# JamesYang007/adelie

Hardware: AMD Instinct MI355X
Metric: lambda-paths/sec (100-lambda grpnet); HBM GB/s vs peak (higher is better)
Workload: dtype f64

## Files before the change

adelie_amd/csrc/kernels.hpp:

```cpp
#pragma once
#include <hip/hip_runtime.h>
#include <cstdint>

namespace ahip {

template <class T>
struct DenseView {
    const T* X;
    int64_t n, p, ld;
};
struct SnpView {
    const uint8_t* bits;
    int64_t n, p, ldb;
};

template <class T>
struct CscView {
    const int64_t* cptr;
    const int32_t* cidx;
    const T* cval;
    const int64_t* rptr;
    const int32_t* rcol;
    const T* rval;
    int64_t n, p, nnz;
// ... 102 lines not shown
    int32_t moff[MAX], m[MAX], noff[MAX], nn[MAX];
    int64_t dst[MAX];
    int32_t count;
};
int64_t gram_batch_work_elems(int64_t n, int count);
template <class T>
void launch_gram_batch(const DenseView<T>& X, const T* w, const int32_t* cols_base, const GramBatch& b, const T* xm_by_col,
                       bool center, T* C_base, int64_t ldc, T* work, hipStream_t s);
template <class T>
void launch_gram_batch_snp(const SnpView& X, const T* impute, const T* w, const int32_t* cols_base, const GramBatch& b,
                           const T* xm_by_col, bool center, T* C_base, int64_t ldc, T* work, hipStream_t s);
struct StripBatch {
    static constexpr int MAX = 8;
    int32_t voff[MAX], m[MAX], c0off[MAX], c0n[MAX], c1off[MAX], c1n[MAX], row0[MAX];
    int64_t dstX[MAX], dstD[MAX];
    int32_t count;
};
int strip_row_tiles(int m);
int64_t strip_work_elems(int64_t n, int count, int m_max);
void set_strip_workgroups(int wgs);
void set_strip_lds(bool on);
template <class T>
void launch_strip_batch(const DenseView<T>& X, const T* w, const int32_t* cols_base, const StripBatch& b, const T* xm_by_col,
                        bool center, T* D_base, T* X_base, int64_t ldc, T* work, hipStream_t s);
void set_small_gram_workgroups(int wgs);
template <class T>
void launch_syrk_batch(const DenseView<T>& X, const T* w, const int32_t* cols_base, const SyrkBatch& b, const T* xm_by_col,
                       bool center, T* C_base, int64_t ldc, T* work, hipStream_t s);
template <class T>
void launch_syrk_batch_snp(const SnpView& X, const T* impute, const T* w, const int32_t* cols_base, const SyrkBatch& b,
                           const T* xm_by_col, bool center, T* C_base, int64_t ldc, T* work, hipStream_t s);
template <class T>
void launch_syrk(const DenseView<T>& X, const T* w, const int32_t* cols, int32_t M, const T* xm_by_col, bool center, T* C,
                   int64_t ldc, T* work, hipStream_t s);
template <class T>
void launch_syrk_snp(const SnpView& X, const T* impute, const T* w, const int32_t* cols, int32_t M, const T* xm_by_col,
                       bool center, T* C, int64_t ldc, T* work, hipStream_t s);
int64_t syrk_work_elems(int64_t n, int64_t M);

template <class T>
void launch_abs_grad(const T* grad, const int64_t* groups, const int64_t* group_sizes, int64_t G, const int32_t* slot,
                     const T* screen_beta, const T* penalty, T one_minus_alpha_lmda, T* abs_grad, hipStream_t s);
template <class T>
void launch_abs_grad_cons(const T* grad, const int64_t* groups, const int64_t* group_sizes, int64_t G, const int32_t* slot, const T* screen_beta,
                          const T* penalty, T one_minus_alpha_lmda, const T* clo, const T* chi, const T* cmu, T* abs_grad,
                          T* mu_out, hipStream_t s);

// ... 212 lines not shown
int launch_panel_step(const DenseView<T>& X, const T* w, T* r, const int32_t* dcol, const T* dlt, const int32_t* nz_dev,
                      const int32_t* cols, int nb, T* part, hipStream_t s);
template <class T>
struct StepTail {
    int32_t* counter;
    int32_t base;
    T* g;
    const T* rsum;
    const T* xm;
};
template <class T>
int launch_panel_step_snp(const SnpView& X, const T* impute, const T* w, T* r, const int32_t* dcol, const T* dlt,
                          const int32_t* nz_dev, const int32_t* cols, int nb, T* part, hipStream_t s,
                          const StepTail<T>* tail = nullptr, bool* tailed = nullptr);
int64_t panel_part_elems(int64_t n);
template <class T>
void launch_la_open_from_grad(const T* grad, const int32_t* cols, int nb, T* g, const T* rsum_src, T* rsum_out, hipStream_t s);
template <class T>
void launch_panel_reduce(const T* part, int nslices, int nb, const int32_t* cols, const T* rsum_dev, const T* xm_by_col,
                         T* gblk, hipStream_t s);
template <class T>
void launch_panel_reduce_ld(const T* part, int64_t part_ld, int nslices, int nb, const int32_t* cols, const T* rsum_dev,
                            const T* xm_by_col, T* gblk, hipStream_t s);
template <class T>
int launch_panel_fused(const CdBlkParams<T>& sp, int j, const DenseView<T>& X, const T* w, T* r, const int32_t* dcol,
                       const T* dlt, const int32_t* nz_dev, const int32_t* cols, int nb, T* part, bool tr, hipStream_t s);
template <class T>
int launch_panel_fused_snp(const CdBlkParams<T>& sp, int j, const SnpView& X, const T* impute, const T* w, T* r,
                           const int32_t* dcol, const T* dlt, const int32_t* nz_dev, const int32_t* cols, int nb, T* part,
                           bool tr, hipStream_t s);
template <class T>
int launch_panel_fused_grp(const CdGrpBlkParams<T>& sp, int j, const DenseView<T>& X, const T* w, T* r, const int32_t* dcol,
                           const T* dlt, const int32_t* nz_dev, const int32_t* cols, int nb, T* part, bool tr, hipStream_t s);
template <class T>
int launch_panel_fused_grp_snp(const CdGrpBlkParams<T>& sp, int j, const SnpView& X, const T* impute, const T* w, T* r,
                               const int32_t* dcol, const T* dlt, const int32_t* nz_dev, const int32_t* cols, int nb,
                               T* part, bool tr, hipStream_t s);
template <class T> void launch_cd_panel_solve(const CdBlkParams<T>& p, int j, hipStream_t s);
template <class T> void launch_center_vars(T* vars, const T* xm, int cnt, bool center, hipStream_t s);
void launch_gather_i32(const int32_t* src, const int32_t* idx, int cnt, int32_t* out, hipStream_t s);
template <class T>
void launch_cd_compact(const T* beta, const T* beta0, const int32_t* vcol, int nv, int32_t* dcols, T* dvals,
                       int32_t* n_delta, hipStream_t s);

template <class T>
struct MultiView {
// ... 138 lines not shown
```

adelie_amd/csrc/kernels_cd_panel.hip:

```cpp
#include "kernels.hpp"
#include "accessors.hpp"
#include "wavered.hpp"
#include "blk_solve_body.hpp"
#include "grp_solve_body.hpp"

namespace ahip {

namespace {

constexpr int PB = 128;
constexpr int PT = 256;

template <class T, int VEC>
struct RawDense { Pack<T, VEC> v; };
struct RawSnp { unsigned byte; };

template <class T, int VEC>
__device__ __forceinline__ RawDense<T, VEC> praw(const DenseAcc<T>& X, int64_t j, int64_t i, int64_t n, bool full) {
    RawDense<T, VEC> r;
    const T* col = X.colptr(j);
    if constexpr (VEC == 1) {
        const T x = col[(full || i < n) ? i : 0];
        r.v.v[0] = (full || i < n) ? x : T(0);
    } else {
// ... 420 lines not shown
            const T* b0 = reinterpret_cast<const T*>(smem_raw);
            const int c = threadIdx.x;
            const T tot = (b0[c] + b0[size_t(5) * RS + c]) + (b0[size_t(10) * RS + c] + b0[size_t(15) * RS + c]);
            T* dst = part + (part_ld > 0 ? int64_t(c) * part_ld + grp : grp * PB + c);
            if (coh) __hip_atomic_store(dst, tot, __ATOMIC_RELAXED, __HIP_MEMORY_SCOPE_AGENT);
            else *dst = tot;
        }
    } else {
        const int64_t slice4 = grp * FS + sub;
        if ((grp + 1) * FS * RS <= n)
            panel_step_body<T, Acc, VEC, true>(X, n, w, r, dcol, dlt, nz, cols, nb, part, part_ld, red, wrs, tid, slice4);
        else
            panel_step_body<T, Acc, VEC, false>(X, n, w, r, dcol, dlt, nz, cols, nb, part, part_ld, red, wrs, tid, slice4);
    }
}

inline int fused_fsa(int64_t ns) {
    if ((ns + 3) / 4 > 250) return 4;
    if (ns <= 250) return 1;
    if ((ns + 1) / 2 <= 250) return 2;
    return 4;
}

template <class T, class Acc, int VEC>
__global__ __launch_bounds__(256 * FS) void panel_fused_kernel(CdBlkParams<T> sp, int j, Acc X, int64_t n,
                                                              const T* __restrict__ w, T* __restrict__ r,
                                                              const int32_t* __restrict__ dcol, const T* __restrict__ dlt,
                                                              const int32_t* __restrict__ nz_dev,
                                                              const int32_t* __restrict__ cols, int nb,
                                                              T* __restrict__ part, int64_t part_ld, int fsa) {
    extern __shared__ __attribute__((aligned(16))) char smem_raw[];
    constexpr int RS = 64 * VEC;
    if (blockIdx.x == 0) {
        if (j < 0) {
            if (threadIdx.x == 0 && sp.part_rsum) {
                const T v = sp.part_rsum[0];
                sp.rsum_out[0] = v;
                sp.rsum_out[1] = v;
            }
            return;
        }
        blk_solve_la_body<T>(sp, j, smem_raw, threadIdx.x);
        return;
    }
    fused_step_part<T, Acc, VEC>(smem_raw, X, n, w, r, dcol, dlt, nz_dev, cols, nb, part, part_ld, fsa);
}
// ... 100 lines not shown
            }
            red[q * PB + c] = sacc;
        }
        __syncthreads();
        if (int(threadIdx.x) < cpw && c < nb) {
            T g = ((red[c] + red[PB + c]) + (red[2 * PB + c] + red[3 * PB + c])) +
                  ((red[4 * PB + c] + red[5 * PB + c]) + (red[6 * PB + c] + red[7 * PB + c]));
            if (sp.tail_xm) g -= sp.tail_rsum[0] * sp.tail_xm[cols[c]];
            sp.tail_g[c] = g;
        }
        if (threadIdx.x == 0) {
            const int d = __hip_atomic_fetch_add(sp.tail_counter + 1, 1, __ATOMIC_RELAXED, __HIP_MEMORY_SCOPE_AGENT);
            if (d == NT - 1) {
                __hip_atomic_store(sp.tail_counter + 1, 0, __ATOMIC_RELAXED, __HIP_MEMORY_SCOPE_AGENT);
                __hip_atomic_store(sp.tail_counter, 0, __ATOMIC_RELAXED, __HIP_MEMORY_SCOPE_AGENT);
            }
        }
    }
}

template <class T, class Acc, int VEC>
int fused_grp_launch(const CdGrpBlkParams<T>& sp, int j, const Acc& acc, int64_t n, const T* w, T* r, const int32_t* dcol,
                     const T* dlt, const int32_t* nz_dev, const int32_t* cols, int nb, T* part, bool tr, hipStream_t s) {
    constexpr int RS = 64 * VEC;
    const int64_t ns = (n + RS - 1) / RS;
    const int fsa = (64 * VEC >= PB) ? fused_fsa(ns) : FS;
    const int64_t nwg = (ns + fsa - 1) / fsa;
    const int64_t part_ld = (64 * VEC >= PB) ? nwg : nwg * FS;
    static bool attr_done = false;
    if (!attr_done) {
        (void)hipFuncSetAttribute(reinterpret_cast<const void*>(panel_fused_grp_kernel<T, Acc, VEC>),
                                  hipFuncAttributeMaxDynamicSharedMemorySize, int(grp_solve_lds_total<T>()));
        attr_done = true;
    }
    hipLaunchKernelGGL((panel_fused_grp_kernel<T, Acc, VEC>), dim3((unsigned)(nwg + 1)), dim3(256 * FS),
                       grp_solve_lds_total<T>(), s, sp, j, acc, n, w, r, dcol, dlt, nz_dev, cols, nb, part,
                       tr ? int64_t(0) : part_ld, fsa);
    return int(part_ld);
}

template <class T, class Acc, int VEC>
int fused_launch(const CdBlkParams<T>& sp, int j, const Acc& acc, int64_t n, const T* w, T* r, const int32_t* dcol,
                 const T* dlt, const int32_t* nz_dev, const int32_t* cols, int nb, T* part, bool tr, hipStream_t s) {
    constexpr int RS = 64 * VEC;
    const int64_t ns = (n + RS - 1) / RS;
    const int fsa = (64 * VEC >= PB) ? fused_fsa(ns) : FS;
    const int64_t nwg = (ns + fsa - 1) / fsa;
    const int64_t part_ld = (64 * VEC >= PB) ? nwg : nwg * FS;
    static bool attr_done = false;
    if (!attr_done) {
        (void)hipFuncSetAttribute(reinterpret_cast<const void*>(panel_fused_kernel<T, Acc, VEC>),
                                  hipFuncAttributeMaxDynamicSharedMemorySize, int(fused_lds<T>()));
        attr_done = true;
    }
    hipLaunchKernelGGL((panel_fused_kernel<T, Acc, VEC>), dim3((unsigned)(nwg + 1)), dim3(256 * FS),
                       fused_lds<T>(), s, sp, j, acc, n, w, r, dcol, dlt, nz_dev, cols, nb, part,
                       tr ? int64_t(0) : part_ld, fsa);
    return int(part_ld);
}

}

template <class T>
int launch_panel_fused(const CdBlkParams<T>& sp, int j, const DenseView<T>& X, const T* w, T* r, const int32_t* dcol,
                       const T* dlt, const int32_t* nz_dev, const int32_t* cols, int nb, T* part, bool tr, hipStream_t s) {
    DenseAcc<T> acc{X.X, X.ld};
    constexpr int V = VecOf<T>::N;
    const bool vecok = (X.ld % V == 0) && ((reinterpret_cast<uintptr_t>(X.X) % 16) == 0);
    if (vecok) return fused_launch<T, DenseAcc<T>, V>(sp, j, acc, X.n, w, r, dcol, dlt, nz_dev, cols, nb, part, tr, s);
    return fused_launch<T, DenseAcc<T>, 1>(sp, j, acc, X.n, w, r, dcol, dlt, nz_dev, cols, nb, part, tr, s);
}
template <class T>
int launch_panel_fused_snp(const CdBlkParams<T>& sp, int j, const SnpView& X, const T* impute, const T* w, T* r,
                           const int32_t* dcol, const T* dlt, const int32_t* nz_dev, const int32_t* cols, int nb, T* part,
                           bool tr, hipStream_t s) {
    SnpAcc<T> acc{X.bits, X.ldb, impute};
    return fused_launch<T, SnpAcc<T>, 4>(sp, j, acc, X.n, w, r, dcol, dlt, nz_dev, cols, nb, part, tr, s);
}

template <class T>
int launch_panel_fused_grp(const CdGrpBlkParams<T>& sp, int j, const DenseView<T>& X, const T* w, T* r, const int32_t* dcol,
                           const T* dlt, const int32_t* nz_dev, const int32_t* cols, int nb, T* part, bool tr, hipStream_t s) {
    DenseAcc<T> acc{X.X, X.ld};
// ... 118 lines not shown
```

adelie_amd/csrc/kernels_strip.hip:

```cpp
#include "gram_common.hpp"
#include "common.hpp"
#include <type_traits>

namespace ahip {

namespace {

constexpr int SGT = 256;
constexpr int SKC = 4;
constexpr int SCH = 4 * SKC;
constexpr int STG = 4;
constexpr int SW = 256;

template <class T, class Acc, bool VECOK, int MT, int TGL>
__device__ __forceinline__ void strip_wave(const Acc& X, const T* __restrict__ w, const int32_t* __restrict__ cols_base,
                                           const StripBatch& b, int y, int wv, int lane, int64_t k0, int64_t k1,
                                           T* __restrict__ P) {
    const int fr = lane & 15, fq = lane >> 4;
    const int m = b.m[y], c0n = b.c0n[y], ncol = c0n + b.c1n[y];
    const T* pa[MT];
    const T* pb[TGL];
    int64_t ja[MT], jb[TGL];
#pragma unroll
    for (int i = 0; i < MT; ++i) {
// ... 98 lines not shown
}

template <class T, class Acc, bool VECOK, int MT>
__global__ __launch_bounds__(SGT, (MT <= 2 ? 2 : 1)) void strip_kernel(Acc X, const T* __restrict__ w,
                                                                      const int32_t* __restrict__ cols_base, StripBatch b,
                                                                      int64_t n, int64_t kchunk, int nsplit,
                                                                      T* __restrict__ part) {
    const int y = blockIdx.y, sp = blockIdx.x;
    const int lane = threadIdx.x & 63;
    const int wv = __builtin_amdgcn_readfirstlane(int(threadIdx.x >> 6));
    const int ncol = b.c0n[y] + b.c1n[y];
    const int tg_live = min(STG, (ncol - wv * 64 + 15) >> 4);
    if (tg_live <= 0 || b.m[y] <= 0) return;
    const int64_t k0 = int64_t(sp) * kchunk, k1 = min(n, k0 + kchunk);
    if (k0 >= k1) return;
    T* P = part + (int64_t(y) * nsplit + sp) * (16 * MT) * SW;
    if (tg_live == 4) strip_wave<T, Acc, VECOK, MT, 4>(X, w, cols_base, b, y, wv, lane, k0, k1, P);
    else if (tg_live == 3) strip_wave<T, Acc, VECOK, MT, 3>(X, w, cols_base, b, y, wv, lane, k0, k1, P);
    else if (tg_live == 2) strip_wave<T, Acc, VECOK, MT, 2>(X, w, cols_base, b, y, wv, lane, k0, k1, P);
    else strip_wave<T, Acc, VECOK, MT, 1>(X, w, cols_base, b, y, wv, lane, k0, k1, P);
}

constexpr int SLP = 18;

template <class Acc, int MT, int TGL>
__device__ __forceinline__ void strip_wave_lt(const Acc& X, const double* __restrict__ w, const int32_t* __restrict__ cols_base,
                                              const StripBatch& b, int y, int wv, int lane, int64_t k0, int64_t k1,
                                              double* __restrict__ P, double* __restrict__ L) {
    using T = double;
    constexpr int NF = MT + TGL;
    const int fr = lane & 15, fq = lane >> 4;
    const int lc = lane >> 3, lp = lane & 7;
    const int m = b.m[y], c0n = b.c0n[y], ncol = c0n + b.c1n[y];
    const T* pg[NF][2];
    int64_t jg[NF][2];
#pragma unroll
    for (int f = 0; f < NF; ++f)
#pragma unroll
        for (int h = 0; h < 2; ++h) {
            const int c16 = h * 8 + lc;
            int64_t j;
            if (f < MT) {
                j = int64_t(cols_base[b.voff[y] + min(f * 16 + c16, m - 1)]);
            } else {
                const int c = min(wv * 64 + (f - MT) * 16 + c16, ncol - 1);
                j = int64_t(c < c0n ? cols_base[b.c0off[y] + c] : cols_base[b.c1off[y] + c - c0n]);
            }
            jg[f][h] = j;
            pg[f][h] = X.colptr(j) + lp * 2;
        }
    typename Mfma<T>::acc_t acc[MT][TGL];
#pragma unroll
    for (int i = 0; i < MT; ++i)
#pragma unroll
        for (int t = 0; t < TGL; ++t)
#pragma unroll
            for (int e = 0; e < 4; ++e) acc[i][t][e] = T(0);

    T g[NF][2][2], fv[NF][SKC], rw[SKC], rwn[SKC];
    auto fetch = [&](int64_t k) {
#pragma unroll
        for (int f = 0; f < NF; ++f)
#pragma unroll
            for (int h = 0; h < 2; ++h) {
                const Pack<T, 2> x = X.template load<2>(pg[f][h], k, jg[f][h]);
                g[f][h][0] = x.v[0];
                g[f][h][1] = x.v[1];
            }
#pragma unroll
        for (int u = 0; u < 2; ++u)
#pragma unroll
            for (int e = 0; e < 2; ++e) rwn[u * 2 + e] = w[k + u * 8 + fq * 2 + e];
    };
    typedef double d2_t __attribute__((ext_vector_type(2)));
    auto park = [&]() {
#pragma unroll
        for (int f = 0; f < NF; ++f)
#pragma unroll
            for (int h = 0; h < 2; ++h) {
                d2_t v = {g[f][h][0], g[f][h][1]};
                *reinterpret_cast<d2_t*>(L + (f * 16 + h * 8 + lc) * SLP + lp * 2) = v;
            }
#pragma unroll
        for (int e = 0; e < SKC; ++e) rw[e] = rwn[e];
    };
    auto frags = [&]() {
#pragma unroll
        for (int f = 0; f < NF; ++f)
#pragma unroll
            for (int u = 0; u < 2; ++u) {
                const d2_t v = *reinterpret_cast<const d2_t*>(L + (f * 16 + fr) * SLP + u * 8 + fq * 2);
                fv[f][u * 2] = v[0];
                fv[f][u * 2 + 1] = v[1];
            }
    };
    auto run = [&]() {
#pragma unroll
        for (int e = 0; e < SKC; ++e) {
            T a[MT];
#pragma unroll
            for (int i = 0; i < MT; ++i) a[i] = fv[i][e] * rw[e];
#pragma unroll
            for (int i = 0; i < MT; ++i)
#pragma unroll
                for (int t = 0; t < TGL; ++t) acc[i][t] = Mfma<T>::run(a[i], fv[MT + t][e], acc[i][t]);
        }
    };
    const int64_t kfull = k0 + ((k1 - k0) / SCH) * SCH;
    int64_t k = k0;
    if (k < kfull) {
        fetch(k);
        while (k < kfull) {
            park();
            fetch((k + 2 * SCH <= kfull) ? k + SCH : k);
            __builtin_amdgcn_fence(__ATOMIC_RELEASE, "wavefront");
            __builtin_amdgcn_wave_barrier();
            __builtin_amdgcn_fence(__ATOMIC_ACQUIRE, "wavefront");
            frags();
            __builtin_amdgcn_fence(__ATOMIC_RELEASE, "wavefront");
            __builtin_amdgcn_wave_barrier();
            run();
            k += SCH;
        }
    }
    if (k < k1) {
#pragma unroll
        for (int u = 0; u < 2; ++u)
#pragma unroll
            for (int e = 0; e < 2; ++e) {
                const int64_t kk = k + u * 8 + fq * 2 + e;
                const bool in = kk < k1;
#pragma unroll
                for (int f = 0; f < NF; ++f) {
                    int64_t j;
                    if (f < MT) {
                        j = int64_t(cols_base[b.voff[y] + min(f * 16 + fr, m - 1)]);
                    } else {
                        const int c = min(wv * 64 + (f - MT) * 16 + fr, ncol - 1);
                        j = int64_t(c < c0n ? cols_base[b.c0off[y] + c] : cols_base[b.c1off[y] + c - c0n]);
                    }
                    fv[f][u * 2 + e] = in ? X.template load<1>(X.colptr(j), kk, j).v[0] : T(0);
                }
                rw[u * 2 + e] = in ? w[kk] : T(0);
            }
        run();
    }
#pragma unroll
    for (int i = 0; i < MT; ++i)
#pragma unroll
        for (int t = 0; t < TGL; ++t)
#pragma unroll
            for (int e = 0; e < 4; ++e) {
                const int row = i * 16 + Mfma<T>::row(lane, e);
                const int col = wv * 64 + t * 16 + fr;
                P[int64_t(row) * SW + col] = acc[i][t][e];
            }
}

template <class Acc, int MT>
__global__ __launch_bounds__(SGT, (MT <= 2 ? 2 : 1)) void strip_lt_kernel(Acc X, const double* __restrict__ w,
                                                                         const int32_t* __restrict__ cols_base, StripBatch b,
                                                                         int64_t n, int64_t kchunk, int nsplit,
                                                                         double* __restrict__ part) {
    __shared__ double lds[4][(MT + STG) * 16 * SLP];
    const int y = blockIdx.y, sp = blockIdx.x;
    const int lane = threadIdx.x & 63;
    const int wv = __builtin_amdgcn_readfirstlane(int(threadIdx.x >> 6));
    const int ncol = b.c0n[y] + b.c1n[y];
    const int tg_live = min(STG, (ncol - wv * 64 + 15) >> 4);
    if (tg_live <= 0 || b.m[y] <= 0) return;
    const int64_t k0 = int64_t(sp) * kchunk, k1 = min(n, k0 + kchunk);
    if (k0 >= k1) return;
    double* P = part + (int64_t(y) * nsplit + sp) * (16 * MT) * SW;
    double* L = &lds[wv][0];
    if (tg_live == 4) strip_wave_lt<Acc, MT, 4>(X, w, cols_base, b, y, wv, lane, k0, k1, P, L);
    else if (tg_live == 3) strip_wave_lt<Acc, MT, 3>(X, w, cols_base, b, y, wv, lane, k0, k1, P, L);
    else if (tg_live == 2) strip_wave_lt<Acc, MT, 2>(X, w, cols_base, b, y, wv, lane, k0, k1, P, L);
    else strip_wave_lt<Acc, MT, 1>(X, w, cols_base, b, y, wv, lane, k0, k1, P, L);
}

template <class T>
__global__ __launch_bounds__(256) void strip_reduce_kernel(const T* __restrict__ part, int nsplit, int rows_pad, StripBatch b,
                                                          const int32_t* __restrict__ cols_base, const T* __restrict__ xm,
                                                          int center, T* __restrict__ D_base, T* __restrict__ X_base,
                                                          int64_t ldc) {
    __shared__ T red[16][17];
    const int y = blockIdx.z, row = blockIdx.y;
    const int m = b.m[y], c0n = b.c0n[y], c1n = b.c1n[y];
    if (row >= m) return;
    const int tc = threadIdx.x & 15, tg = threadIdx.x >> 4;
    const int col = blockIdx.x * 16 + tc;
    const int have = b.row0[y];
    const int cc = col - c0n;
    const bool live = col < c0n + c1n;
    const bool skip = !live || (cc >= 0 && cc > have + row);
    T s = T(0);
    if (!skip) {
        const int64_t stride = int64_t(rows_pad) * SW;
        const T* base = part + int64_t(y) * nsplit * stride + int64_t(row) * SW + col;
        int sp = tg;
        for (; sp + 48 < nsplit; sp += 64) {
// ... 34 lines not shown
}

constexpr int kStripWgsDefault = 192;
thread_local int t_strip_wgs = kStripWgsDefault;
thread_local bool t_strip_lds = true;

}

void set_strip_workgroups(int wgs) { t_strip_wgs = wgs < 1 ? kStripWgsDefault : wgs; }
void set_strip_lds(bool on) { t_strip_lds = on; }

int strip_row_tiles(int m) { return m <= 16 ? 1 : (m <= 32 ? 2 : (m <= 48 ? 3 : (m <= 64 ? 4 : 0))); }

int64_t strip_work_elems(int64_t n, int count, int m_max) {
    int ns;
    int64_t kc;
    strip_shape(n, count, 1024, ns, kc);
    const int mt = strip_row_tiles(m_max);
    return int64_t(count) * ns * 16 * (mt ? mt : 4) * SW;
}

template <class T>
void launch_strip_batch(const DenseView<T>& Xv, const T* w, const int32_t* cols_base, const StripBatch& b, const T* xm_by_col,
                        bool center, T* D_base, T* X_base, int64_t ldc, T* work, hipStream_t s) {
    if (b.count <= 0) return;
    int mx = 0;
    for (int y = 0; y < b.count; ++y) mx = std::max(mx, int(b.m[y]));
    const int MTv = strip_row_tiles(mx);
    if (MTv == 0) throw make_core_error("internal: strip build of more than 64 rows.");
    DenseAcc<T> acc{Xv.X, Xv.ld};
    const bool vecok = (Xv.ld % VecOf<T>::N == 0) && ((reinterpret_cast<uintptr_t>(Xv.X) % 16) == 0);
    int nsplit;
    int64_t kchunk;
    strip_shape(Xv.n, b.count, std::min(t_strip_wgs, 1024), nsplit, kchunk);
    const dim3 grid((unsigned)nsplit, (unsigned)b.count);
#define AHIP_STRIP(VOK, MTV)                                                                                            \
    hipLaunchKernelGGL((strip_kernel<T, DenseAcc<T>, VOK, MTV>), grid, dim3(SGT), 0, s, acc, w, cols_base, b, Xv.n, kchunk, \
                       nsplit, work)
    bool done = false;
    if constexpr (std::is_same<T, double>::value) {
        if (vecok && t_strip_lds) {
#define AHIP_STRIP_LT(MTV)                                                                                              \
    hipLaunchKernelGGL((strip_lt_kernel<DenseAcc<double>, MTV>), grid, dim3(SGT), 0, s, acc, w, cols_base, b, Xv.n, kchunk, \
                       nsplit, work)
            if (MTv == 1) AHIP_STRIP_LT(1);
            else if (MTv == 2) AHIP_STRIP_LT(2);
            else if (MTv == 3) AHIP_STRIP_LT(3);
            else AHIP_STRIP_LT(4);
#undef AHIP_STRIP_LT
            done = true;
        }
    }
    if (!done) {
        if (MTv == 1) { if (vecok) AHIP_STRIP(true, 1); else AHIP_STRIP(false, 1); }
        else if (MTv == 2) { if (vecok) AHIP_STRIP(true, 2); else AHIP_STRIP(false, 2); }
        else if (MTv == 3) { if (vecok) AHIP_STRIP(true, 3); else AHIP_STRIP(false, 3); }
        else { if (vecok) AHIP_STRIP(true, 4); else AHIP_STRIP(false, 4); }
    }
#undef AHIP_STRIP
    hipLaunchKernelGGL((strip_reduce_kernel<T>), dim3(16, (unsigned)mx, (unsigned)b.count), dim3(256), 0, s, work, nsplit,
                       16 * MTv, b, cols_base, xm_by_col, center ? 1 : 0, D_base, X_base, ldc);
}

template void launch_strip_batch<double>(const DenseView<double>&, const double*, const int32_t*, const StripBatch&,
                                         const double*, bool, double*, double*, int64_t, double*, hipStream_t);
template void launch_strip_batch<float>(const DenseView<float>&, const float*, const int32_t*, const StripBatch&, const float*,
                                        bool, float*, float*, int64_t, float*, hipStream_t);

}
```

adelie_amd/csrc/solver_builds.hpp:

```cpp
    adelie_hip_design* D = nullptr;
    hipStream_t st = nullptr;
    idx n, p, G;
    std::vector<idx> groups, group_sizes;
    std::vector<T> penalty;
    std::vector<T> penalty2;
    bool has_pen2 = false;
    std::vector<T> h_spen2;
    T alpha, min_ratio;
    size_t lmda_path_size, max_screen_size, max_active_size;
    T pivot_subset_ratio;
    size_t pivot_subset_min;
    T pivot_slack_ratio;
    int screen_rule;
    size_t max_iters;
    T tol, adev_tol, ddev_tol, newton_tol;
    size_t newton_max_iters;
    bool early_exit_, setup_lmda_max, setup_lmda_path, intercept;
    int glm_kind;
    adelie_hip_poll_fn poll;
    void* poll_user;
    const adelie_hip_result* live = nullptr;
    bool cov_mode = false;
    T rdev_tol = 0;
    DevBuf<T> d_covv, d_zero;
// ... 422 lines not shown
                hipEvent_t e = next_event();
                AHIP_CHECK(hipEventRecord(e, st2));
                x_ev[size_t(j)] = e;
            }
            k.nb_prev = nbp; k.nb = nb; k.ver = w_version;
            ++n_cross_blocks;
        }
    }
    bool strip_builds = true;
    int strip_max_m = 128;
    std::vector<hipEvent_t> strip_pool, strip_ev;
    std::vector<int> strip_built;
    size_t strip_used = 0;
    int64_t n_strip_builds = 0;
    hipEvent_t next_strip_event() {
        if (strip_used == strip_pool.size()) {
            hipEvent_t e;
            AHIP_CHECK(hipEventCreateWithFlags(&e, hipEventDisableTiming));
            strip_pool.push_back(e);
        }
        return strip_pool[strip_used++];
    }
    bool strips_apply() const { return strip_builds && dense() && !is_glm() && D->std_center == nullptr; }
    DevBuf<T> d_Draw;
    template <class NbOf, class ColsOf>
    void build_stale_strips(int nblk, std::vector<int32_t>& tab_nb, std::vector<uint64_t>& tab_ver, std::vector<XKey>* xtab,
                            T* pool, T* xpool, NbOf nb_of, ColsOf cols_of, T* rot_dst = nullptr, const idx* rlist = nullptr,
                            bool force_main = false) {
        strip_ev.assign(size_t(nblk), nullptr);
        strip_used = 0;
        strip_built.clear();
        if (!strips_apply()) return;
        const int SL = cd_block_size();
        const bool side = !force_main && side_grams && st2 != nullptr;
        hipStream_t gs = side ? st2 : st;
        bool first = true;
        const int32_t* cols_base = cols_of(0);
        StripBatch sb{};
        int js[StripBatch::MAX];
        bool ent_d[StripBatch::MAX] = {}, ent_x[StripBatch::MAX] = {};
        auto flush = [&]() {
            if (sb.count == 0) return;
            if (side && first) {
                if (pass_e0_valid) {
                    AHIP_CHECK(hipStreamWaitEvent(st2, pass_e0, 0));
                } else {
                    hipEvent_t e0 = next_strip_event();
                    AHIP_CHECK(hipEventRecord(e0, st));
                    AHIP_CHECK(hipStreamWaitEvent(st2, e0, 0));
                }
                first = false;
            }
            int mx = 0;
            for (int y = 0; y < sb.count; ++y) mx = std::max(mx, int(sb.m[y]));
            T* work = (side ? d_work_gram2 : d_work_gram).reserve(size_t(strip_work_elems(n, sb.count, mx)));
            t_gram.begin(gs);
            launch_strip_batch<T>(D->dense<T>(), cur_w, cols_base, sb, cur_xm, intercept, pool, xpool, SL, work, gs);
            if (rot_dst)
                for (int y = 0; y < sb.count; ++y)
                    if (ent_d[y] && (y == 0 || js[y - 1] != js[y]))
                        rotate_block(rlist, js[y], rot_dst + size_t(js[y]) * SL * SL, side ? 1 : 0, pool + size_t(js[y]) * SL * SL);
            t_gram.end(gs);
            hipEvent_t e = nullptr;
            if (side) {
                e = next_strip_event();
                AHIP_CHECK(hipEventRecord(e, st2));
            }
            for (int y = 0; y < sb.count; ++y) {
                const int j = js[y];
                strip_ev[size_t(j)] = e;
                if (ent_d[y]) {
                    tab_nb[size_t(j)] = nb_of(j);
                    tab_ver[size_t(j)] = w_version;
                }
                if (ent_x[y] && xtab && j > 0) {
                    XKey& key = (*xtab)[size_t(j)];
                    key.nb_prev = nb_of(j - 1); key.nb = nb_of(j); key.ver = w_version;
                }
                cnt.gram_flops += 2.0 * double(n) * double(sb.m[y]) * double(sb.c0n[y] + sb.c1n[y]);
                cnt.n_gram_col_reads += sb.m[y] + sb.c0n[y] + sb.c1n[y];
// ... 95 lines not shown
```

adelie_amd/csrc/solver_panel.hpp:

```cpp
    void run_block_passes(const CdParams<T>& cp, CdScalars<T>& sc, T* r_stale = nullptr) {
        const int B = cd_block_size();
        if (r_stale) {
            d_beta_ref.reserve(size_t(cp.nv) + 8);
            AHIP_CHECK(hipMemcpyAsync(d_beta_ref.p, cp.beta, size_t(cp.nv) * sizeof(T), hipMemcpyDeviceToDevice, st));
        }
        int64_t n_pass = 0;
        d_blk.reserve(1);
        d_Dbuf.reserve(size_t(2) * B * B);
        d_dlt.reserve(B);
        d_didx.reserve(B);
        CdBlkState<T> bs{};
        bs.rsq = sc.rsq;
        bs.resid_sum = sc.resid_sum;
        bs.cm = 0;
        bs.n_updates = 0;
        bs.active_size = sc.active_size;
        bs.status = CD_OK;
        d_blk.upload(&bs, 1, st);
        CdBlkParams<T> bp{};
        bp.nv = cp.nv; bp.C = cp.C; bp.ldc = cp.ldc; bp.vars = cp.vars; bp.xmean = cp.xmean; bp.spen = cp.spen; bp.spen2 = cp.spen2;
        bp.beta = cp.beta; bp.g = cp.g; bp.is_active = cp.is_active; bp.active_set = cp.active_set;
        bp.l1 = cp.lmda * cp.alpha; bp.l2 = cp.lmda * (T(1) - cp.alpha);
        bp.max_active_size = cp.max_active_size;
        bp.Dbuf = d_Dbuf.p; bp.dlt = d_dlt.p; bp.didx = d_didx.p; bp.st = d_blk.p;
// ... 205 lines not shown
                const int32_t* dc = ps < 0 ? d_dcolblk.p : d_la_dcol.p + size_t(ps) * SL;
                const T* dl = ps < 0 ? d_dlt.p : d_la_dlt.p + size_t(ps) * SL;
                const int32_t* nzp = ps < 0 ? &d_blk.p->nz : d_la_nz.p + ps;
                T* part_out = d_part2.p + part2_half;
                if (time_panel) t_step.begin(st);
                if (dense())
                    prev_ld = launch_panel_fused<T>(op, -1, D->dense<T>(), cur_w, r_dev, dc, dl, nzp, cols_all, nb_of(0), part_out, true, st);
                else
                    prev_ld = launch_panel_fused_snp<T>(op, -1, D->snp(), static_cast<const T*>(D->impute), cur_w, r_dev, dc, dl, nzp,
                                                        cols_all, nb_of(0), part_out, true, st);
                if (time_panel) t_step.end(st);
                cnt.n_panel_cols += nb_of(0);
            } else {
                const int nb01 = nb_of(0) + (nblk > 1 ? nb_of(1) : 0);
                const int ps = pending_slot;
                if (time_panel) t_step.begin(st);
                const int nsl = panel_step(cur_w, r_dev, ps < 0 ? d_dcolblk.p : d_la_dcol.p + size_t(ps) * SL,
                                           ps < 0 ? d_dlt.p : d_la_dlt.p + size_t(ps) * SL,
                                           ps < 0 ? &d_blk.p->nz : d_la_nz.p + ps, cols_all, nb01);
                if (time_panel) t_step.end(st);
                launch_panel_reduce<T>(d_part.p, nsl, nb01, cols_all, &d_blk.p->resid_sum, xm_c, d_la_g.p, st);
                cnt.n_panel_cols += nb01;
            }
            build_stale_strips(nblk, tab_nb, tab_ver, screen_pass ? &xscr_key : &xact_key, pool, xpool, nb_of, cols_of);
            build_stale_blocks(nblk, tab_nb, tab_ver, pool, nb_of, cols_of);
            build_stale_cross(nblk, screen_pass ? xscr_key : xact_key, xpool, nb_of, cols_of);
            merge_strip_events(true);
            pass_e0_valid = false;
            for (int j = 0; j < nblk; ++j) {
                const int slot = j & 1, pslot = slot ^ 1;
                bp.gblk = d_la_g.p + size_t(slot) * B;
                bp.part = (fuse_reduce && prev_ld > 0) ? d_part2.p + size_t((j - 1) & 1) * part2_half : nullptr;
                bp.part_ld = 0;
                bp.part_n = prev_ld;
                bp.part_rsum = xm_c ? d_la_rsum.p + slot : nullptr;
                prev_ld = 0;
                bp.Dptr = pool + size_t(j) * SL * SL;
                bp.Cprev = j > 0 ? xpool + size_t(j) * SL * SL : nullptr;
                bp.pdlt = d_la_dlt.p + size_t(pslot) * SL;
                bp.ppos = d_la_dpos.p + size_t(pslot) * SL;
                bp.pnz = d_la_nz.p + pslot;
                bp.dlt = d_la_dlt.p + size_t(slot) * SL;
                bp.dcol = d_la_dcol.p + size_t(slot) * SL;
                bp.dpos = d_la_dpos.p + size_t(slot) * SL;
                bp.nz_out = d_la_nz.p + slot;
                bp.rsum_out = d_la_rsum.p + slot;
                bp.pdd = d_la_dd.p + size_t(pslot) * SL;
// ... 662 lines not shown
                if (time_panel) t_step.begin(st);
                launch_panel_fused_grp<T>(op, -1, D->dense<T>(), cur_w, r_dev, ps < 0 ? d_dcolblk.p : d_la_dcol.p + size_t(ps) * SL,
                                          ps < 0 ? d_dlt.p : d_la_dlt.p + size_t(ps) * SL, ps < 0 ? &d_blk.p->nz : d_la_nz.p + ps,
                                          cols_all, nb_of(0), d_part2.p, true, st);
                if (time_panel) t_step.end(st);
                cnt.n_panel_cols += nb_of(0);
            } else {
                const int nv0 = nb_of(0), nv1 = nblk > 1 ? nb_of(1) : 0;
                const int ps = pending_slot;
                if (time_panel) t_step.begin(st);
                const int nsl = panel_step(cur_w, r_dev, ps < 0 ? d_dcolblk.p : d_la_dcol.p + size_t(ps) * SL,
                                           ps < 0 ? d_dlt.p : d_la_dlt.p + size_t(ps) * SL,
                                           ps < 0 ? &d_blk.p->nz : d_la_nz.p + ps, cols_all, nv0 + nv1);
                if (time_panel) t_step.end(st);
                launch_panel_reduce<T>(d_part.p, nsl, nv0, cols_all, &d_blk.p->resid_sum, xm_c, d_la_g.p, st);
                if (nv1 > 0)
                    launch_panel_reduce<T>(d_part.p + size_t(nv0) * size_t(nsl), nsl, nv1, cols_all + nv0, &d_blk.p->resid_sum,
                                           xm_c, d_la_g.p + SL, st);
                cnt.n_panel_cols += nv0 + nv1;
            }
            if (strips_apply() && !multi()) {
                T* raw = group_rot ? d_Draw.reserve(size_t(2) * maxblk * SL * SL) + (screen_pass ? size_t(0) : maxblk * SL * SL) : pool;
                build_stale_strips(nblk, tab_nb, tab_ver, screen_pass ? &xscr_key : &xact_key, raw, xpool, nb_of, cols_of,
                                   group_rot ? pool : nullptr, screen_pass ? nullptr : act_host.data());
            } else {
                strip_ev.clear();
            }
            rot_on = group_rot;
            rot_list = screen_pass ? nullptr : act_host.data();
            build_stale_blocks(nblk, tab_nb, tab_ver, pool, nb_of, cols_of);
            rot_on = false;
            build_stale_cross(nblk, screen_pass ? xscr_key : xact_key, xpool, nb_of, cols_of);
            merge_strip_events(true);
            pass_e0_valid = false;
            if (screen_pass) join_uv();
            int prev_ld = 0;
            const bool next_corr = bp.rot && !multi();
            if (next_corr) d_la_corr.reserve(size_t(2) * SL);
            bool prev_made_corr = false;
            for (int j = 0; j < nblk; ++j) {
                const int slot = j & 1, pslot = slot ^ 1;
                bp.gblk = d_la_g.p + size_t(slot) * SL;
                bp.Dptr = pool + size_t(j) * SL * SL;
                bp.Cprev = j > 0 ? xpool + size_t(j) * SL * SL : nullptr;
                bp.corr_in = (prev_made_corr && j > 0) ? d_la_corr.p + size_t(pslot) * SL : nullptr;
                const bool fused_j = !(j == 0 && !fr_open);
                bp.Cnext = (next_corr && fused_j && j + 1 < nblk) ? xpool + size_t(j + 1) * SL * SL : nullptr;
// ... 261 lines not shown
```

Measured before the change: 3.970.

## Share strip A-tile across waves via LDS and cap strip grid beside fused panel

```diff
diff --git a/adelie_amd/csrc/kernels.hpp b/adelie_amd/csrc/kernels.hpp
--- a/adelie_amd/csrc/kernels.hpp
+++ b/adelie_amd/csrc/kernels.hpp
@@ -148,7 +148,7 @@
 void set_strip_lds(bool on);
 template <class T>
 void launch_strip_batch(const DenseView<T>& X, const T* w, const int32_t* cols_base, const StripBatch& b, const T* xm_by_col,
-                        bool center, T* D_base, T* X_base, int64_t ldc, T* work, hipStream_t s);
+                        bool center, T* D_base, T* X_base, int64_t ldc, T* work, hipStream_t s, int max_wgs = 0);
 void set_small_gram_workgroups(int wgs);
 template <class T>
 void launch_syrk_batch(const DenseView<T>& X, const T* w, const int32_t* cols_base, const SyrkBatch& b, const T* xm_by_col,
@@ -407,6 +407,7 @@
 template <class T>
 void launch_panel_reduce_ld(const T* part, int64_t part_ld, int nslices, int nb, const int32_t* cols, const T* rsum_dev,
                             const T* xm_by_col, T* gblk, hipStream_t s);
+int panel_fused_workgroups(int64_t n, int vec);
 template <class T>
 int launch_panel_fused(const CdBlkParams<T>& sp, int j, const DenseView<T>& X, const T* w, T* r, const int32_t* dcol,
                        const T* dlt, const int32_t* nz_dev, const int32_t* cols, int nb, T* part, bool tr, hipStream_t s);
diff --git a/adelie_amd/csrc/kernels_cd_panel.hip b/adelie_amd/csrc/kernels_cd_panel.hip
--- a/adelie_amd/csrc/kernels_cd_panel.hip
+++ b/adelie_amd/csrc/kernels_cd_panel.hip
@@ -466,6 +466,12 @@
     return 4;
 }
 
+inline int64_t fused_step_wgs(int64_t n, int vec, int& fsa) {
+    const int64_t rs = 64 * vec, ns = (n + rs - 1) / rs;
+    fsa = (rs >= PB) ? fused_fsa(ns) : FS;
+    return (ns + fsa - 1) / fsa;
+}
+
 template <class T, class Acc, int VEC>
 __global__ __launch_bounds__(256 * FS) void panel_fused_kernel(CdBlkParams<T> sp, int j, Acc X, int64_t n,
                                                               const T* __restrict__ w, T* __restrict__ r,
@@ -612,10 +618,8 @@
 template <class T, class Acc, int VEC>
 int fused_grp_launch(const CdGrpBlkParams<T>& sp, int j, const Acc& acc, int64_t n, const T* w, T* r, const int32_t* dcol,
                      const T* dlt, const int32_t* nz_dev, const int32_t* cols, int nb, T* part, bool tr, hipStream_t s) {
-    constexpr int RS = 64 * VEC;
-    const int64_t ns = (n + RS - 1) / RS;
-    const int fsa = (64 * VEC >= PB) ? fused_fsa(ns) : FS;
-    const int64_t nwg = (ns + fsa - 1) / fsa;
+    int fsa;
+    const int64_t nwg = fused_step_wgs(n, VEC, fsa);
     const int64_t part_ld = (64 * VEC >= PB) ? nwg : nwg * FS;
     static bool attr_done = false;
     if (!attr_done) {
@@ -632,10 +636,8 @@
 template <class T, class Acc, int VEC>
 int fused_launch(const CdBlkParams<T>& sp, int j, const Acc& acc, int64_t n, const T* w, T* r, const int32_t* dcol,
                  const T* dlt, const int32_t* nz_dev, const int32_t* cols, int nb, T* part, bool tr, hipStream_t s) {
-    constexpr int RS = 64 * VEC;
-    const int64_t ns = (n + RS - 1) / RS;
-    const int fsa = (64 * VEC >= PB) ? fused_fsa(ns) : FS;
-    const int64_t nwg = (ns + fsa - 1) / fsa;
+    int fsa;
+    const int64_t nwg = fused_step_wgs(n, VEC, fsa);
     const int64_t part_ld = (64 * VEC >= PB) ? nwg : nwg * FS;
     static bool attr_done = false;
     if (!attr_done) {
@@ -649,6 +651,11 @@
     return int(part_ld);
 }
 
+}
+
+int panel_fused_workgroups(int64_t n, int vec) {
+    int fsa;
+    return int(fused_step_wgs(n, vec, fsa)) + 1;
 }
 
 template <class T>
diff --git a/adelie_amd/csrc/kernels_strip.hip b/adelie_amd/csrc/kernels_strip.hip
--- a/adelie_amd/csrc/kernels_strip.hip
+++ b/adelie_amd/csrc/kernels_strip.hip
@@ -144,33 +144,97 @@
 }
 
 constexpr int SLP = 18;
+constexpr int SQ = 2;
+constexpr int SGC = SQ * SGT;
+constexpr int SLB = STG * 16 * SLP;
+
+__device__ __forceinline__ void strip_wg_barrier() {
+    __builtin_amdgcn_fence(__ATOMIC_RELEASE, "workgroup");
+    __builtin_amdgcn_s_barrier();
+    __builtin_amdgcn_fence(__ATOMIC_ACQUIRE, "workgroup");
+}
+
+typedef double strip_d2_t __attribute__((ext_vector_type(2)));
+
+template <class Acc, int MT>
+struct StripAShare {
+    static constexpr int NAW = (2 * MT + 3) / 4;
+    const double* pg[NAW];
+    int64_t jg[NAW];
+    int off[NAW];
+    bool on[NAW];
+    double g[NAW][2];
+    __device__ __forceinline__ void init(const Acc& X, const int32_t* __restrict__ cols_base, const StripBatch& b, int y, int wv,
+                                         int lane) {
+        const int lc = lane >> 3, lp = lane & 7, m = b.m[y];
+#pragma unroll
+        for (int u = 0; u < NAW; ++u) {
+            const int idx = wv + 4 * u;
+            on[u] = idx < 2 * MT;
+            const int c = min(idx, 2 * MT - 1) * 8 + lc;
+            const int64_t j = int64_t(cols_base[b.voff[y] + min(c, m - 1)]);
+            jg[u] = j;
+            pg[u] = X.colptr(j) + lp * 2;
+            off[u] = c * SLP + lp * 2;
+        }
+    }
+    __device__ __forceinline__ void fetch(const Acc& X, int64_t k) {
+#pragma unroll
+        for (int u = 0; u < NAW; ++u)
+            if (on[u]) {
+                const Pack<double, 2> x = X.template load<2>(pg[u], k, jg[u]);
+                g[u][0] = x.v[0];
+                g[u][1] = x.v[1];
+            }
+    }
+    __device__ __forceinline__ void park(double* __restrict__ A) const {
+#pragma unroll
+        for (int u = 0; u < NAW; ++u)
+            if (on[u]) {
+                strip_d2_t v = {g[u][0], g[u][1]};
+                *reinterpret_cast<strip_d2_t*>(A + off[u]) = v;
+            }
+    }
+};
+
+template <class Acc, int MT>
+__device__ __forceinline__ void strip_wave_feed(const Acc& X, const int32_t* __restrict__ cols_base, const StripBatch& b, int y,
+                                                int wv, int lane, int64_t k0, int nmine, int nmax, double* __restrict__ A) {
+    StripAShare<Acc, MT> as;
+    as.init(X, cols_base, b, y, wv, lane);
+    int64_t k = k0;
+    if (nmine > 0) as.fetch(X, k);
+    for (int c = 0; c < nmax; ++c) {
+        if (c < nmine) {
+            as.park(A + (c & 1) * (MT * 16 * SLP));
+            as.fetch(X, (c + 1 < nmine) ? k + SCH : k);
+            k += SCH;
+        }
+        strip_wg_barrier();
+    }
+}
 
 template <class Acc, int MT, int TGL>
 __device__ __forceinline__ void strip_wave_lt(const Acc& X, const double* __restrict__ w, const int32_t* __restrict__ cols_base,
-                                              const StripBatch& b, int y, int wv, int lane, int64_t k0, int64_t k1,
-                                              double* __restrict__ P, double* __restrict__ L) {
+                                              const StripBatch& b, int y, int wv, int lane, int64_t k0, int64_t k1, int nmine,
+                                              int nmax, double* __restrict__ P, double* __restrict__ L, double* __restrict__ A) {
     using T = double;
-    constexpr int NF = MT + TGL;
     const int fr = lane & 15, fq = lane >> 4;
     const int lc = lane >> 3, lp = lane & 7;
     const int m = b.m[y], c0n = b.c0n[y], ncol = c0n + b.c1n[y];
-    const T* pg[NF][2];
-    int64_t jg[NF][2];
-#pragma unroll
-    for (int f = 0; f < NF; ++f)
+    const T* pg[TGL][2];
+    int64_t jg[TGL][2];
+#pragma unroll
+    for (int t = 0; t < TGL; ++t)
 #pragma unroll
         for (int h = 0; h < 2; ++h) {
-            const int c16 = h * 8 + lc;
-            int64_t j;
-            if (f < MT) {
-                j = int64_t(cols_base[b.voff[y] + min(f * 16 + c16, m - 1)]);
-            } else {
-                const int c = min(wv * 64 + (f - MT) * 16 + c16, ncol - 1);
-                j = int64_t(c < c0n ? cols_base[b.c0off[y] + c] : cols_base[b.c1off[y] + c - c0n]);
-            }
-            jg[f][h] = j;
-            pg[f][h] = X.colptr(j) + lp * 2;
-        }
+            const int c = min(wv * 64 + t * 16 + h * 8 + lc, ncol - 1);
+            const int64_t j = int64_t(c < c0n ? cols_base[b.c0off[y] + c] : cols_base[b.c1off[y] + c - c0n]);
+            jg[t][h] = j;
+            pg[t][h] = X.colptr(j) + lp * 2;
+        }
+    StripAShare<Acc, MT> as;
+    as.init(X, cols_base, b, y, wv, lane);
     typename Mfma<T>::acc_t acc[MT][TGL];
 #pragma unroll
     for (int i = 0; i < MT; ++i)
@@ -179,81 +243,83 @@
 #pragma unroll
             for (int e = 0; e < 4; ++e) acc[i][t][e] = T(0);
 
-    T g[NF][2][2], fv[NF][SKC], rw[SKC], rwn[SKC];
+    T g[TGL][2][2], fv[MT + TGL][2], rw[SKC], rwn[SKC];
     auto fetch = [&](int64_t k) {
-#pragma unroll
-        for (int f = 0; f < NF; ++f)
+        as.fetch(X, k);
+#pragma unroll
+        for (int t = 0; t < TGL; ++t)
 #pragma unroll
             for (int h = 0; h < 2; ++h) {
-                const Pack<T, 2> x = X.template load<2>(pg[f][h], k, jg[f][h]);
-                g[f][h][0] = x.v[0];
-                g[f][h][1] = x.v[1];
+                const Pack<T, 2> x = X.template load<2>(pg[t][h], k, jg[t][h]);
+                g[t][h][0] = x.v[0];
+                g[t][h][1] = x.v[1];
             }
 #pragma unroll
         for (int u = 0; u < 2; ++u)
 #pragma unroll
             for (int e = 0; e < 2; ++e) rwn[u * 2 + e] = w[k + u * 8 + fq * 2 + e];
     };
-    typedef double d2_t __attribute__((ext_vector_type(2)));
-    auto park = [&]() {
-#pragma unroll
-        for (int f = 0; f < NF; ++f)
+    auto park = [&](double* __restrict__ Ac) {
+        as.park(Ac);
+#pragma unroll
+        for (int t = 0; t < TGL; ++t)
 #pragma unroll
             for (int h = 0; h < 2; ++h) {
-                d2_t v = {g[f][h][0], g[f][h][1]};
-                *reinterpret_cast<d2_t*>(L + (f * 16 + h * 8 + lc) * SLP + lp * 2) = v;
+                strip_d2_t v = {g[t][h][0], g[t][h][1]};
+                *reinterpret_cast<strip_d2_t*>(L + (t * 16 + h * 8 + lc) * SLP + lp * 2) = v;
             }
 #pragma unroll
         for (int e = 0; e < SKC; ++e) rw[e] = rwn[e];
     };
-    auto frags = [&]() {
-#pragma unroll
-        for (int f = 0; f < NF; ++f)
-#pragma unroll
-            for (int u = 0; u < 2; ++u) {
-                const d2_t v = *reinterpret_cast<const d2_t*>(L + (f * 16 + fr) * SLP + u * 8 + fq * 2);
-                fv[f][u * 2] = v[0];
-                fv[f][u * 2 + 1] = v[1];
-            }
-    };
-    auto run = [&]() {
-#pragma unroll
-        for (int e = 0; e < SKC; ++e) {
+    auto frags = [&](const double* __restrict__ Ac, int u) {
+#pragma unroll
+        for (int f = 0; f < MT + TGL; ++f) {
+            const double* src = f < MT ? Ac + (f * 16 + fr) * SLP : L + ((f - MT) * 16 + fr) * SLP;
+            const strip_d2_t v = *reinterpret_cast<const strip_d2_t*>(src + u * 8 + fq * 2);
+            fv[f][0] = v[0];
+            fv[f][1] = v[1];
+        }
+    };
+    auto run = [&](int u) {
+#pragma unroll
+        for (int e = 0; e < 2; ++e) {
             T a[MT];
 #pragma unroll
-            for (int i = 0; i < MT; ++i) a[i] = fv[i][e] * rw[e];
+            for (int i = 0; i < MT; ++i) a[i] = fv[i][e] * rw[u * 2 + e];
 #pragma unroll
             for (int i = 0; i < MT; ++i)
 #pragma unroll
                 for (int t = 0; t < TGL; ++t) acc[i][t] = Mfma<T>::run(a[i], fv[MT + t][e], acc[i][t]);
         }
     };
-    const int64_t kfull = k0 + ((k1 - k0) / SCH) * SCH;
     int64_t k = k0;
-    if (k < kfull) {
-        fetch(k);
-        while (k < kfull) {
-            park();
-            fetch((k + 2 * SCH <= kfull) ? k + SCH : k);
+    if (nmine > 0) fetch(k);
+    for (int c = 0; c < nmax; ++c) {
+        double* Ac = A + (c & 1) * (MT * 16 * SLP);
+        if (c < nmine) {
+            park(Ac);
+            fetch((c + 1 < nmine) ? k + SCH : k);
+        }
+        strip_wg_barrier();
+        if (c < nmine) {
+            frags(Ac, 0);
+            run(0);
+            frags(Ac, 1);
             __builtin_amdgcn_fence(__ATOMIC_RELEASE, "wavefront");
             __builtin_amdgcn_wave_barrier();
-            __builtin_amdgcn_fence(__ATOMIC_ACQUIRE, "wavefront");
-            frags();
-            __builtin_amdgcn_fence(__ATOMIC_RELEASE, "wavefront");
-            __builtin_amdgcn_wave_barrier();
-            run();
+            run(1);
             k += SCH;
         }
     }
     if (k < k1) {
 #pragma unroll
-        for (int u = 0; u < 2; ++u)
+        for (int u = 0; u < 2; ++u) {
 #pragma unroll
             for (int e = 0; e < 2; ++e) {
                 const int64_t kk = k + u * 8 + fq * 2 + e;
                 const bool in = kk < k1;
 #pragma unroll
-                for (int f = 0; f < NF; ++f) {
+                for (int f = 0; f < MT + TGL; ++f) {
                     int64_t j;
                     if (f < MT) {
                         j = int64_t(cols_base[b.voff[y] + min(f * 16 + fr, m - 1)]);
@@ -261,11 +327,12 @@
                         const int c = min(wv * 64 + (f - MT) * 16 + fr, ncol - 1);
                         j = int64_t(c < c0n ? cols_base[b.c0off[y] + c] : cols_base[b.c1off[y] + c - c0n]);
                     }
-                    fv[f][u * 2 + e] = in ? X.template load<1>(X.colptr(j), kk, j).v[0] : T(0);
+                    fv[f][e] = in ? X.template load<1>(X.colptr(j), kk, j).v[0] : T(0);
                 }
                 rw[u * 2 + e] = in ? w[kk] : T(0);
             }
-        run();
+            run(u);
+        }
     }
 #pragma unroll
     for (int i = 0; i < MT; ++i)
@@ -280,25 +347,44 @@
 }
 
 template <class Acc, int MT>
-__global__ __launch_bounds__(SGT, (MT <= 2 ? 2 : 1)) void strip_lt_kernel(Acc X, const double* __restrict__ w,
-                                                                         const int32_t* __restrict__ cols_base, StripBatch b,
-                                                                         int64_t n, int64_t kchunk, int nsplit,
-                                                                         double* __restrict__ part) {
-    __shared__ double lds[4][(MT + STG) * 16 * SLP];
-    const int y = blockIdx.y, sp = blockIdx.x;
+__global__ __launch_bounds__(SGC) void strip_lt_kernel(Acc X, const double* __restrict__ w,
+                                                       const int32_t* __restrict__ cols_base, StripBatch b, int64_t n,
+                                                       int64_t kchunk, int nsplit, double* __restrict__ part) {
+    __shared__ double ldsB[SQ * 4][SLB];
+    __shared__ double ldsA[SQ][2 * MT * 16 * SLP];
     const int lane = threadIdx.x & 63;
-    const int wv = __builtin_amdgcn_readfirstlane(int(threadIdx.x >> 6));
-    const int ncol = b.c0n[y] + b.c1n[y];
-    const int tg_live = min(STG, (ncol - wv * 64 + 15) >> 4);
-    if (tg_live <= 0 || b.m[y] <= 0) return;
-    const int64_t k0 = int64_t(sp) * kchunk, k1 = min(n, k0 + kchunk);
-    if (k0 >= k1) return;
-    double* P = part + (int64_t(y) * nsplit + sp) * (16 * MT) * SW;
-    double* L = &lds[wv][0];
-    if (tg_live == 4) strip_wave_lt<Acc, MT, 4>(X, w, cols_base, b, y, wv, lane, k0, k1, P, L);
-    else if (tg_live == 3) strip_wave_lt<Acc, MT, 3>(X, w, cols_base, b, y, wv, lane, k0, k1, P, L);
-    else if (tg_live == 2) strip_wave_lt<Acc, MT, 2>(X, w, cols_base, b, y, wv, lane, k0, k1, P, L);
-    else strip_wave_lt<Acc, MT, 1>(X, w, cols_base, b, y, wv, lane, k0, k1, P, L);
+    const int wq = __builtin_amdgcn_readfirstlane(int(threadIdx.x >> 6));
+    const int q = wq >> 2, wv = wq & 3;
+    const int items = b.count * nsplit, stride = int(gridDim.x) * SQ;
+    auto chunks_of = [&](int id) {
+        if (id >= items || b.m[id / nsplit] <= 0) return 0;
+        const int64_t k0 = int64_t(id % nsplit) * kchunk, k1 = min(n, k0 + kchunk);
+        return k1 > k0 ? int((k1 - k0) / SCH) : 0;
+    };
+    for (int first = int(blockIdx.x) * SQ; first < items; first += stride) {
+        int nmax = 0;
+#pragma unroll
+        for (int u = 0; u < SQ; ++u) nmax = max(nmax, chunks_of(first + u));
+        const int id = first + q;
+        const int y = id < items ? id / nsplit : 0, sp = id < items ? id % nsplit : 0;
+        const int64_t k0 = int64_t(sp) * kchunk, k1 = min(n, k0 + kchunk);
+        const int ncol = b.c0n[y] + b.c1n[y];
+        const int tg_live = min(STG, (ncol - wv * 64 + 15) >> 4);
+        double* A = &ldsA[q][0];
+        if (id >= items || b.m[y] <= 0 || k0 >= k1) {
+            for (int c = 0; c < nmax; ++c) strip_wg_barrier();
+        } else {
+            const int nmine = int((k1 - k0) / SCH);
+            double* P = part + (int64_t(y) * nsplit + sp) * (16 * MT) * SW;
+            double* L = &ldsB[wq][0];
+            if (tg_live == 4) strip_wave_lt<Acc, MT, 4>(X, w, cols_base, b, y, wv, lane, k0, k1, nmine, nmax, P, L, A);
+            else if (tg_live == 3) strip_wave_lt<Acc, MT, 3>(X, w, cols_base, b, y, wv, lane, k0, k1, nmine, nmax, P, L, A);
+            else if (tg_live == 2) strip_wave_lt<Acc, MT, 2>(X, w, cols_base, b, y, wv, lane, k0, k1, nmine, nmax, P, L, A);
+            else if (tg_live == 1) strip_wave_lt<Acc, MT, 1>(X, w, cols_base, b, y, wv, lane, k0, k1, nmine, nmax, P, L, A);
+            else strip_wave_feed<Acc, MT>(X, cols_base, b, y, wv, lane, k0, nmine, nmax, A);
+        }
+        strip_wg_barrier();
+    }
 }
 
 template <class T>
@@ -379,7 +465,7 @@
 
 template <class T>
 void launch_strip_batch(const DenseView<T>& Xv, const T* w, const int32_t* cols_base, const StripBatch& b, const T* xm_by_col,
-                        bool center, T* D_base, T* X_base, int64_t ldc, T* work, hipStream_t s) {
+                        bool center, T* D_base, T* X_base, int64_t ldc, T* work, hipStream_t s, int max_wgs) {
     if (b.count <= 0) return;
     int mx = 0;
     for (int y = 0; y < b.count; ++y) mx = std::max(mx, int(b.m[y]));
@@ -397,9 +483,11 @@
     bool done = false;
     if constexpr (std::is_same<T, double>::value) {
         if (vecok && t_strip_lds) {
+            int wgs = (nsplit * b.count + SQ - 1) / SQ;
+            if (max_wgs > 0 && wgs > max_wgs) wgs = max_wgs;
 #define AHIP_STRIP_LT(MTV)                                                                                              \
-    hipLaunchKernelGGL((strip_lt_kernel<DenseAcc<double>, MTV>), grid, dim3(SGT), 0, s, acc, w, cols_base, b, Xv.n, kchunk, \
-                       nsplit, work)
+    hipLaunchKernelGGL((strip_lt_kernel<DenseAcc<double>, MTV>), dim3((unsigned)wgs), dim3(SGC), 0, s, acc, w, cols_base, b, \
+                       Xv.n, kchunk, nsplit, work)
             if (MTv == 1) AHIP_STRIP_LT(1);
             else if (MTv == 2) AHIP_STRIP_LT(2);
             else if (MTv == 3) AHIP_STRIP_LT(3);
@@ -420,8 +508,8 @@
 }
 
 template void launch_strip_batch<double>(const DenseView<double>&, const double*, const int32_t*, const StripBatch&,
-                                         const double*, bool, double*, double*, int64_t, double*, hipStream_t);
+                                         const double*, bool, double*, double*, int64_t, double*, hipStream_t, int);
 template void launch_strip_batch<float>(const DenseView<float>&, const float*, const int32_t*, const StripBatch&, const float*,
-                                        bool, float*, float*, int64_t, float*, hipStream_t);
-
-}
+                                        bool, float*, float*, int64_t, float*, hipStream_t, int);
+
+}
diff --git a/adelie_amd/csrc/solver_builds.hpp b/adelie_amd/csrc/solver_builds.hpp
--- a/adelie_amd/csrc/solver_builds.hpp
+++ b/adelie_amd/csrc/solver_builds.hpp
@@ -468,11 +468,24 @@
         return strip_pool[strip_used++];
     }
     bool strips_apply() const { return strip_builds && dense() && !is_glm() && D->std_center == nullptr; }
+    static constexpr int kStripMinFreeCus = 32;
+    int cu_count = 0;
+    int strip_grid_cap() {
+        if (cu_count == 0) {
+            int dev = 0;
+            AHIP_CHECK(hipGetDevice(&dev));
+            AHIP_CHECK(hipDeviceGetAttribute(&cu_count, hipDeviceAttributeMultiprocessorCount, dev));
+        }
+        constexpr int V = int(16 / sizeof(T));
+        const bool vecok = (D->ld % V == 0) && ((reinterpret_cast<uintptr_t>(D->X) % 16) == 0);
+        const int free_cus = cu_count - panel_fused_workgroups(n, vecok ? V : 1);
+        return free_cus >= kStripMinFreeCus ? free_cus : 0;
+    }
     DevBuf<T> d_Draw;
     template <class NbOf, class ColsOf>
     void build_stale_strips(int nblk, std::vector<int32_t>& tab_nb, std::vector<uint64_t>& tab_ver, std::vector<XKey>* xtab,
                             T* pool, T* xpool, NbOf nb_of, ColsOf cols_of, T* rot_dst = nullptr, const idx* rlist = nullptr,
-                            bool force_main = false) {
+                            bool force_main = false, bool beside_fused = false) {
         strip_ev.assign(size_t(nblk), nullptr);
         strip_used = 0;
         strip_built.clear();
@@ -480,6 +493,7 @@
         const int SL = cd_block_size();
         const bool side = !force_main && side_grams && st2 != nullptr;
         hipStream_t gs = side ? st2 : st;
+        const int max_wgs = (side && beside_fused) ? strip_grid_cap() : 0;
         bool first = true;
         const int32_t* cols_base = cols_of(0);
         StripBatch sb{};
@@ -501,7 +515,7 @@
             for (int y = 0; y < sb.count; ++y) mx = std::max(mx, int(sb.m[y]));
             T* work = (side ? d_work_gram2 : d_work_gram).reserve(size_t(strip_work_elems(n, sb.count, mx)));
             t_gram.begin(gs);
-            launch_strip_batch<T>(D->dense<T>(), cur_w, cols_base, sb, cur_xm, intercept, pool, xpool, SL, work, gs);
+            launch_strip_batch<T>(D->dense<T>(), cur_w, cols_base, sb, cur_xm, intercept, pool, xpool, SL, work, gs, max_wgs);
             if (rot_dst)
                 for (int y = 0; y < sb.count; ++y)
                     if (ent_d[y] && (y == 0 || js[y - 1] != js[y]))
diff --git a/adelie_amd/csrc/solver_panel.hpp b/adelie_amd/csrc/solver_panel.hpp
--- a/adelie_amd/csrc/solver_panel.hpp
+++ b/adelie_amd/csrc/solver_panel.hpp
@@ -251,7 +251,8 @@
                 launch_panel_reduce<T>(d_part.p, nsl, nb01, cols_all, &d_blk.p->resid_sum, xm_c, d_la_g.p, st);
                 cnt.n_panel_cols += nb01;
             }
-            build_stale_strips(nblk, tab_nb, tab_ver, screen_pass ? &xscr_key : &xact_key, pool, xpool, nb_of, cols_of);
+            build_stale_strips(nblk, tab_nb, tab_ver, screen_pass ? &xscr_key : &xact_key, pool, xpool, nb_of, cols_of, nullptr,
+                               nullptr, false, true);
             build_stale_blocks(nblk, tab_nb, tab_ver, pool, nb_of, cols_of);
             build_stale_cross(nblk, screen_pass ? xscr_key : xact_key, xpool, nb_of, cols_of);
             merge_strip_events(true);
@@ -960,7 +961,7 @@
             if (strips_apply() && !multi()) {
                 T* raw = group_rot ? d_Draw.reserve(size_t(2) * maxblk * SL * SL) + (screen_pass ? size_t(0) : maxblk * SL * SL) : pool;
                 build_stale_strips(nblk, tab_nb, tab_ver, screen_pass ? &xscr_key : &xact_key, raw, xpool, nb_of, cols_of,
-                                   group_rot ? pool : nullptr, screen_pass ? nullptr : act_host.data());
+                                   group_rot ? pool : nullptr, screen_pass ? nullptr : act_host.data(), false, true);
             } else {
                 strip_ev.clear();
             }
```

Result: slower. 3.472 (-12.6%).
